# patello/azul_deep_reinforcement_learning

Hardware: AMD Instinct MI355X
Metric: Azul env steps/sec (random-agent self-play), bit-exact vs CPU (higher is better)
Workload: dtype u8/u32 (+f64 sampling)

## Files before the change

### azul_deep_reinforcement_learning_amd/csrc/azul_common.hpp

```cpp
#pragma once
#include <stdint.h>

typedef uint32_t u32;
typedef int32_t  i32;
typedef uint64_t u64;
typedef int64_t  i64;

#if !defined(__HIPCC__)
#error "libazulhip's headers are gfx950 device code: compile with hipcc --offload-arch=gfx950"
#endif
#include <hip/hip_runtime.h>
#define AZ_FN __device__ __forceinline__
#define AZ_MEMBER_FN __attribute__((device)) __forceinline__
#define AZ_UNLIKELY(x) __builtin_expect(!!(x), 0)

namespace wv {
AZ_FN u32 lane() { return __builtin_amdgcn_mbcnt_hi(~0u, __builtin_amdgcn_mbcnt_lo(~0u, 0u)); }

template <class A, class B> struct same_type { static constexpr bool value = false; };
template <class A> struct same_type<A, A> { static constexpr bool value = true; };
constexpr bool LOCKSTEP_EMULATION = same_type<decltype(__builtin_amdgcn_s_memtime()), unsigned long long>::value;
template <int SIMM16> struct HwReg { static constexpr int value = SIMM16; };
template <class R> AZ_FN u32 getreg(R)
{
    if constexpr (LOCKSTEP_EMULATION) return 0u;
    else return __builtin_amdgcn_s_getreg(R::value);
}
AZ_FN u32 hw_id() { return getreg(HwReg<(4 | (31 << 11))>()); }
AZ_FN u32 hw_xcc_id() { return getreg(HwReg<(20 | (31 << 11))>()); }
constexpr int PRIO_BLOCK = 128;
AZ_FN void set_prio(bool hi) { if (hi) __builtin_amdgcn_s_setprio(1); else __builtin_amdgcn_s_setprio(0); }
}

namespace az {

enum { ST_OK = 0, ST_ILLEGAL_MOVE = 1, ST_GAME_ENDED = 2, ST_STUCK = 3, ST_BAD_ACTION = 4, ST_BOX_EMPTY = 5,
       ST_TRUNCATED = 6  };
enum { POOL_RANDOM = 0, POOL_LID = 1 };
#ifndef AZ_DRAW_MARGIN
#define AZ_DRAW_MARGIN 8192ull
#endif
enum { T_ROWS = 31, T_BINADES = 8, T_STRIDE = 9 , T_PAIRS = T_ROWS * T_STRIDE };

enum { SEG_MASK = 0, SEG_SAMPLE, SEG_MOVE, SEG_AFTERMOVE, SEG_TAIL, SEG_NEWROUND, SEG_SCORE, SEG_RESET, SEG_LOOP, SEG_COUNT };
constexpr int AZ_PROF_SLOTS = 48;
enum { WCNT_ROUND_END = 0, WCNT_DEAL, WCNT_RESET, WCNT_COUNT };
constexpr int AZ_WAVE_REC_WORDS = 8;
#if defined(AZ_PROFILE_SEGMENTS)
struct SegProf { u64 last; u64 acc[SEG_COUNT]; u32 cnt[WCNT_COUNT]; };
#define AZ_COUNT(which, cond) do { if (prof_) prof_->cnt[which] += (u32)__popcll(__builtin_amdgcn_ballot_w64(cond)) >> 5; } while (0)
struct WaveStamps { u64 entry, loop_start, loop_end; };
#define AZ_WAVE_STAMP(field) (wstamps.field = __builtin_amdgcn_s_memtime())
#define AZ_STAMP(seg) do { if (prof_) { u64 now_ = __builtin_amdgcn_s_memtime(); prof_->acc[seg] += now_ - prof_->last; prof_->last = now_; } } while (0)
#else
struct SegProf { int unused; };
#define AZ_STAMP(seg) do { } while (0)
#define AZ_COUNT(which, cond) do { } while (0)
#define AZ_WAVE_STAMP(field) do { } while (0)
#endif

struct Rules {
    u32 first_player;
    u32 tile_pool;
};

constexpr u32 column_board_c(int col)
{
    u32 m = 0;
    for (int j = 0; j < 5; j++) m |= 1u << (5 * j + ((col - j + 5) % 5));
    return m;
}
static_assert(column_board_c(0) == 0x222201u && column_board_c(4) == 0x111110u, "column boards");

AZ_FN i32 floor_penalty(u32 floor_tiles)
{
// ... 53 lines not shown
```

### azul_deep_reinforcement_learning_amd/csrc/azul_kernels.hip

```cpp
#include <hip/hip_runtime.h>
#include <math.h>
#include <stdio.h>
#include <stdlib.h>
#include <string.h>

#include <mutex>
#include <string>
#include <vector>

#include "../../include/azul_hip.h"
#include "azul_common.hpp"
#include "azul_tables.hpp"

using namespace az;

#include "azul_selfplay_kernels.hpp"

#include "azul_x_kernels.hpp"

#include "azul_policy.hpp"
#include "azul_rollout2.hpp"
#include "azul_learner.hpp"

struct azul_batch {
// ... 78 lines not shown
    for (void *p : bufs) if (p) (void)hipFree(p);
    if (b->ev0) (void)hipEventDestroy(b->ev0);
    if (b->ev1) (void)hipEventDestroy(b->ev1);
    for (hipEvent_t e : b->lev) (void)hipEventDestroy(e);
    if (b->call_pin) (void)hipHostFree(b->call_pin);
    delete b;
}

static int batch_alloc(azul_batch *b, int n_games, int first_player, int tile_pool)
{
    HIP_TRY(hipGetDevice(&b->device));
    const size_t N = (size_t)n_games;
    const size_t RB = (size_t)b->rec_bytes;
    b->d.n = (u32)n_games;
    b->d.rules.first_player = (u32)first_player;
    b->d.rules.tile_pool = (u32)tile_pool;
    b->d.draw_margin = AZ_DRAW_MARGIN;
    HIP_TRY(hipMalloc((void **)&b->d.state, N * RB));
    HIP_TRY(hipMalloc((void **)&b->d.mt, N * 624 * sizeof(u32)));
    HIP_TRY(hipMalloc((void **)&b->d.mtpos, N * sizeof(u32)));
    HIP_TRY(hipMalloc((void **)&b->d.episodes, N * sizeof(u64)));
    HIP_TRY(hipMalloc((void **)&b->d.stuck, N * sizeof(u32)));
    HIP_TRY(hipMalloc((void **)&b->d.stat_sum, N * 10 * sizeof(double)));
    HIP_TRY(hipMalloc((void **)&b->d.prof, AZ_PROF_SLOTS * sizeof(u64)));
    HIP_TRY(hipMemset(b->d.prof, 0, AZ_PROF_SLOTS * sizeof(u64)));
#if defined(AZ_PROFILE_SEGMENTS)
    HIP_TRY(hipMalloc((void **)&b->d.wave_prof, (N + 1) / 2 * AZ_WAVE_REC_WORDS * sizeof(u64)));
    HIP_TRY(hipMemset(b->d.wave_prof, 0, (N + 1) / 2 * AZ_WAVE_REC_WORDS * sizeof(u64)));
#endif
    {
        const int rows = 5 * (b->displays + 1) + 1;
        std::vector<double> hX((size_t)rows * T_STRIDE * 2);
        if (!build_sample_pairs(rows, hX.data())) return fail(AZUL_ERR_INVALID, "weight-table decomposition check failed on this host");
        HIP_TRY(hipMalloc((void **)&b->Tx, hX.size() * sizeof(double)));
        HIP_TRY(hipMemcpy(b->Tx, hX.data(), hX.size() * sizeof(double), hipMemcpyHostToDevice));
        b->d.tab = (const double2 *)b->Tx;
    }
    HIP_TRY(hipMemset(b->d.state, 0, N * RB));
    HIP_TRY(hipMemset(b->d.mt, 0, N * 624 * sizeof(u32)));
    {
        std::vector<u32> pos(N, 624u);
        HIP_TRY(hipMemcpy(b->d.mtpos, pos.data(), N * sizeof(u32), hipMemcpyHostToDevice));
    }
    HIP_TRY(hipMemset(b->d.episodes, 0, N * sizeof(u64)));
    HIP_TRY(hipMemset(b->d.stuck, 0, N * sizeof(u32)));
    HIP_TRY(hipMemset(b->d.stat_sum, 0, N * 10 * sizeof(double)));
    HIP_TRY(hipEventCreate(&b->ev0));
    HIP_TRY(hipEventCreate(&b->ev1));
    return AZUL_SUCCESS;
}

int azul_batch_create(azul_batch_t **out, int n_games, int first_player, int tile_pool)
{
    return azul_batch_create_players(out, n_games, 2, first_player, tile_pool);
}

int azul_batch_create_players(azul_batch_t **out, int n_games, int players, int first_player, int tile_pool)
{
    return azul_batch_create_rules(out, n_games, players, first_player, tile_pool, 0u);
}

int azul_batch_create_rules(azul_batch_t **out, int n_games, int players, int first_player, int tile_pool, unsigned rule_flags)
{
    if (!out || n_games <= 0) return fail(AZUL_ERR_INVALID, "azul_batch_create: bad arguments");
    if (players < 2 || players > 4) return fail(AZUL_ERR_INVALID, "players must be 2, 3 or 4");
    if (first_player < 0 || first_player > players) return fail(AZUL_ERR_RULE, "first_player must be 0 (Random) or 1 .. players");
// ... 1410 lines not shown
```

### azul_deep_reinforcement_learning_amd/csrc/azul_rules_x.hpp

```cpp
#pragma once
#include "azul_selfplay2.hpp"
#include "azul_env2.hpp"

namespace azx {
using namespace az;
using namespace az2;

enum { XPOOL_RANDOM = 0, XPOOL_LID = 1, XPOOL_BAG = 2 };

struct RulesX {
    u32 first_player;
    u32 pool;
    u32 end_bonus;
    u32 short_deal;
};

template <u32 D>
struct Dim {
    static constexpr u32 S = D + 1;
    static constexpr u32 Q = 5 * S;
    static constexpr u32 NA = 6 * Q;
    static constexpr u32 NW = Q > 32 ? 2 : 1;
    static constexpr u32 NL = (NA + 63) / 64;
    static constexpr u32 TROWS = Q + 1;
// ... 611 lines not shown
            if (o.action) o.action[o.e] = av;
            if (o.reward) o.reward[o.e] = 0;
            if (o.packed) o.packed[o.e] = pk;
            if (o.done) o.done[o.e] = (uint8_t)dn;
        }
        if (o.rec) gx_store(g, o.rec + o.e * (u32)AZUL_RECORD_BYTES_WIDE, l);
    }
}

template <u32 P, u32 D, int OUT, bool PAD, bool BITS>
AZ_FN u32 selfplay_step_x(GX<P, D> &g, const RulesX &rules, const KX<D> &K, Rng2 &r, const Tab2 &T, u64 margin, Counters2 &cnt,
                          const Out2 &o, bool &dead, SegProf *prof_ = nullptr)
{
    (void)prof_;
    AZ_STAMP(SEG_LOOP);
    const K2 &k = K.k;
    const u32 l = k.l;
    const bool hard = r.pos + 2u > 624u;
    u32 wa, wb;
    {
        const u32 i = hard ? 622u : r.pos;
        wa = r.tlds[i]; wb = r.tlds[i + 1u];
    }
    MaskX<D> m;
    legal_mask_x(g, K, m);
    u32 pre[7];
    pre[0] = 0;
#pragma unroll
    for (u32 rr = 0; rr < 6u; rr++) pre[rr + 1] = pre[rr] + row_count<D>(m, rr);
    const u32 J = pre[1], L = pre[6];
    const bool nomove = (L == 0u) | (g.eog != 0u);
    const u32 M = L - J, Mc = M ? M : 256u, Jc = J < Dim<D>::TROWS ? J : Dim<D>::TROWS - 1u;
    const u32 kbase = M ? J : 0u;
    const double u01 = ((double)(wa >> 5) * 67108864.0 + (double)(wb >> 6)) * (1.0 / 9007199254740992.0);
    const double2 fs = T.fs[9u * Jc + 31u - (u32)__builtin_clz(Mc)];
    if (OUT == 1 || (OUT == 2 && o.mask)) store_mask_x<D, (PAD && OUT == 1)>(o, m, l);
    if ((OUT == 1 && BITS) || (OUT == 2 && o.maskbits)) store_maskbits_x<D>(o, m, l);
    AZ_STAMP(SEG_MASK);
    const double sJ = fs.y;
    const double total = ((double)M + fs.x) + 0.0;
    double u = u01;
    double x = u * total;
    double d = x - sJ;
    u32 fl = (u32)d;
    double fr = d - (double)fl;
    u32 kg = kbase + fl + 1u;
    bool edge = !(__builtin_fabs(fr - 0.5) < 0.5 - 1e-9) | (kg > L);
    r.pos += 2u;
    bool any_nomove = false;
    if (AZ_UNLIKELY(wave_any(hard | edge | nomove))) {
        r.pos -= (hard | nomove) ? 2u : 0u;
        if (hard & !nomove) {
            const bool one = r.pos == 623u;
            const u32 last = r.tlds[623];
            lds_sync();
            rng2_twist(r, l);
            const u32 t0 = r.tlds[0], t1 = r.tlds[1];
            wa = one ? last : t0; wb = one ? t0 : t1;
            r.pos = one ? 1u : 2u;
            u = ((double)(wa >> 5) * 67108864.0 + (double)(wb >> 6)) * (1.0 / 9007199254740992.0);
            x = u * total;
            d = x - sJ; fl = (u32)d; fr = d - (double)fl;
            kg = kbase + fl + 1u;
            edge = !(__builtin_fabs(fr - 0.5) < 0.5 - 1e-9) | (kg > L);
        }
        if (edge & !nomove) {
            const double sT = M ? sJ : T.fs[9u * Jc].y;
            kg = sample_slow2(T, M ? x : u * (sT + 0.0), sT, J, M, L);
        }
        any_nomove = wave_any(nomove);
    }
    Choice<D> ch;
    pick_action_x<D>(m, pre, kg, k, ch);
    AZ_STAMP(SEG_SAMPLE);

    u32 ret = 0;
    if (AZ_UNLIKELY(any_nomove)) {
        if (nomove) {
            cnt.stuck_add += 1u;
            {
                MaskX<D> none;
#pragma unroll
                for (u32 rr = 0; rr < 6u; rr++)
#pragma unroll
                    for (u32 ww = 0; ww < Dim<D>::NW; ww++) { none.m[rr][ww] = 0u; none.bit[rr][ww] = 0u; }
                if (OUT == 1 || (OUT == 2 && o.mask)) store_mask_x<D, (PAD && OUT == 1)>(o, none, l);
                if ((OUT == 1 && BITS) || (OUT == 2 && o.maskbits)) store_maskbits_x<D>(o, none, l);
            }
            outputs_x<P, D, OUT>(g, o, -1, 2u, l);
            const u32 st0 = restart_x(g, rules, r, margin, K);
            ret = st0 ? (0x100u | st0) : 2u;
        }
        dead |= (ret & 0x100u) != 0u;
        AZ_STAMP(SEG_RESET);
    }
    if (!nomove) {
        do_move_x(g, ch.s, ch.c, ch.row, rules.pool != (u32)XPOOL_RANDOM, K);
        sources_x(g);
        AZ_STAMP(SEG_MOVE);
        const bool eor = (g.B0 | g.B1) == 0u;
        g.cur = eor ? g.cur : (g.cur < P ? g.cur + 1u : 1u);
        u32 st = ST_OK;
// ... 77 lines not shown
struct XOp {
    int op;
    const i32 *actions;
    const uint8_t *active;
    const uint8_t *mask_in;
    i32 *actions_out;
    uint8_t *status;
    uint8_t *mask;
    float *obs;
    int persp;
    uint8_t *flags;
    double *stats;
    uint8_t *player;
    uint8_t *rng_dirty;
    uint8_t *rec_out;
    u32 *pos_out;
    i32 *next_action;
    u32 pos_set;
    u32 first, count;
};

struct XTraj {
    int n_steps;
    uint8_t *mask; u64 *maskbits; i32 *action; i32 *reward; uint8_t *done; uint8_t *rec; u32 *packed;
    u32 mask_stride;
};

AZ_FN bool xop_draws(int op) { return op == XOP_INIT || op == XOP_NEW_ROUND || op == XOP_STEP || op == XOP_RANDOM_ACTION || op == XOP_SAMPLE_MASK; }

template <u32 D>
AZ_FN void stage_tab_x(const double2 *tab, double2 *tab_lds, u32 lane)
{
    for (u32 i = lane; i < Dim<D>::TROWS * (u32)T_STRIDE; i += 64u) tab_lds[i] = tab[i];
    lds_sync();
}

template <u32 D>
AZ_FN void store_mask_bytes_x(const MaskX<D> &m, uint8_t *row, u32 l)
{
    row += l;
#pragma unroll
    for (u32 rr = 0; rr < 6u; rr++) {
        if (l < (Dim<D>::Q < 32u ? Dim<D>::Q : 32u)) row[Dim<D>::Q * rr] = (uint8_t)m.bit[rr][0];
        if (Dim<D>::NW > 1) { if (l < Dim<D>::Q - 32u) row[Dim<D>::Q * rr + 32u] = (uint8_t)m.bit[rr][Dim<D>::NW - 1]; }
    }
}

template <u32 P, u32 D>
AZ_FN void open_game_x(GX<P, D> &g, KX<D> &K, const uint8_t *rec, u32 l)
{
    kx_init(K);
    gx_load(g, rec, l);
    prime_x(g, K);
}

AZ_FN void open_stream_x(Rng2 &r, Counters2 &cnt, const XBatchDev &b, u32 gi, u32 *lds, u32 l)
{
    rng2_open(r, b.mt + (size_t)gi * 624u, lds, b.mtpos[gi], l);
    counters2_open(cnt, b.episodes + gi, b.stuck + gi, b.stat_sum + (size_t)gi * 10, l);
}
AZ_FN void close_stream_x(Rng2 &r, const Counters2 &cnt, const XBatchDev &b, u32 gi, u32 l)
{
    rng2_close(r, b.mt + (size_t)gi * 624u, b.mtpos + gi, l);
    counters2_close(cnt, l);
}

// ... 77 lines not shown
        if (dirty_state) gx_store(g, rec, l);
        if (a.next_action && use_rng && st == ST_OK && r.pos + 2u <= 624u) {
            const u32 keep = r.pos;
            MaskX<D> m;
            legal_mask_x(g, K, m);
            spec = random_agent_x<D>(m, r, tab, K.k);
            r.pos = keep;
        }
        if (use_rng) rng2_close(r, gmt, b.mtpos + gi, l);
        rdirty = r.dirty;
    }
    if (a.next_action && l == 0u) a.next_action[oi] = spec;
    if (a.rng_dirty && l == 0u) a.rng_dirty[oi] = (uint8_t)rdirty;
    if (a.status && act && l == 0u) a.status[oi] = (uint8_t)st;
    if (a.rec_out) gx_store(g, a.rec_out + (size_t)oi * AZUL_RECORD_BYTES_WIDE, l);
    if (a.pos_out && l == 0u) a.pos_out[oi] = b.mtpos[gi];
    if (a.mask) {
        MaskX<D> m;
        legal_mask_x(g, K, m);
        store_mask_bytes_x<D>(m, a.mask + (size_t)oi * Dim<D>::NA, l);
    }
    if (a.obs) observe_x(g, (u32)a.persp < P ? (u32)a.persp : mex(g), a.obs + (size_t)oi * obs_size<P, D>(), l);
    if (a.flags) {
        const u32 f = ((g.B0 | g.B1) == 0u ? AZUL_FLAG_END_OF_ROUND : 0) | (g.over ? AZUL_FLAG_END_OF_GAME : 0) | (g.eog ? AZUL_FLAG_ENDED_FLAG : 0);
        if (l == 0u) a.flags[oi] = (uint8_t)f;
    }
    if (a.stats) {
        if (l == 0u) for (u32 q = 0; q < 10u; q++) a.stats[(size_t)oi * 10 + q] = game_stat_x(g, q);
    }
    if (a.player && l == 0u) a.player[oi] = (uint8_t)g.cur;
}

template <u32 P, u32 D, int OUT, bool PAD, bool BITS>
AZ_FN void selfplay_body_x(const XBatchDev &b, const XTraj &t, u32 wave_id, u32 (*mt_lds)[624], u32 (*mtt_lds)[624], double2 *tab_lds)
{
    const u32 lane = wv::lane(), l = lane & 31u, half = lane >> 5;
    stage_tab_x<D>(b.tab, tab_lds, lane);
    const u32 gi = wave_id * 2u + half;
    if (gi >= b.n) return;
    uint8_t *rec = b.state + (size_t)gi * AZUL_RECORD_BYTES_WIDE;
    KX<D> K;
    const Tab2 tab = {tab_lds};
    GX<P, D> g;
    open_game_x(g, K, rec, l);
    Rng2 r;
    u32 *gmt = b.mt + (size_t)gi * 624u;
    rng2_open(r, gmt, mt_lds[half], b.mtpos[gi], l);
    rng2_attach_tempered(r, mtt_lds[half], l);
    Counters2 cnt;
    counters2_open(cnt, b.episodes + gi, b.stuck + gi, b.stat_sum + (size_t)gi * 10, l);
    Out2 o = {t.mask, t.maskbits, t.action, t.reward, t.done, t.packed, t.rec, t.mask_stride, gi,
              l == 0u ? (u32 *)t.action : (l == 1u ? (u32 *)t.reward : t.packed)};
    bool dead = false;
#if defined(AZ_PROFILE_SEGMENTS)
    SegProf prof;
    for (int q = 0; q < SEG_COUNT; q++) prof.acc[q] = 0;
    prof.last = __builtin_amdgcn_s_memtime();
    SegProf *pp = &prof;
#else
    SegProf *pp = nullptr;
#endif
    u32 turn = wv::hw_id() & 1u;
#pragma unroll 1
    for (int s0 = 0; s0 < t.n_steps; s0 += wv::PRIO_BLOCK) {
        wv::set_prio(turn != 0u);
        turn ^= 1u;
        const int s1 = s0 + wv::PRIO_BLOCK < t.n_steps ? s0 + wv::PRIO_BLOCK : t.n_steps;
#pragma unroll 1
        for (int s = s0; s < s1; s++) {
            if (!dead) selfplay_step_x<P, D, OUT, PAD, BITS>(g, b.rules, K, r, tab, b.draw_margin, cnt, o, dead, pp);
            else {
                cnt.stuck_add += 1u;
                {
                    MaskX<D> none;
#pragma unroll
// ... 447 lines not shown
```

### azul_deep_reinforcement_learning_amd/csrc/azul_selfplay2.hpp

```cpp
#pragma once
#include "azul_common.hpp"

namespace az2 {
using namespace az;

AZ_FN u32 wlane() { return wv::lane(); }
AZ_FN bool upper() { return (wlane() & 32u) != 0u; }
AZ_FN u32 hsel(u64 b) { return upper() ? (u32)(b >> 32) : (u32)b; }
AZ_FN u32 hb(bool p) { return hsel(__builtin_amdgcn_ballot_w64(p)); }
AZ_FN u32 hread(u32 v, u32 idx) { return (u32)__builtin_amdgcn_ds_bpermute((int)((idx << 2) | ((wlane() & 32u) << 2)), (int)v); }
AZ_FN u32 hbcast(u32 v, u32 idx) { return hread(v, idx); }
AZ_FN u32 hread4(u32 v, u32 idx, u32 h4) { return (u32)__builtin_amdgcn_ds_bpermute((int)((idx << 2) | h4), (int)v); }
template <u32 IDX>
AZ_FN u32 hbcast_c(u32 v)
{
    u32 a = (u32)__builtin_amdgcn_readlane((int)v, (int)IDX), b = (u32)__builtin_amdgcn_readlane((int)v, (int)(IDX + 32u));
    return upper() ? b : a;
}
AZ_FN bool wave_any(bool p) { return __builtin_amdgcn_ballot_w64(p) != 0ull; }
AZ_FN double hread_d(double v, u32 idx)
{
    u64 b = (u64)__double_as_longlong(v);
    u32 lo = hread((u32)b, idx), hi = hread((u32)(b >> 32), idx);
    return __longlong_as_double((long long)(((u64)hi << 32) | lo));
// ... 271 lines not shown
}
#endif

struct Mask2 {
    u32 m[6];
    u32 bit[6];
    u32 B;
};

AZ_FN u32 ok_board2(u32 cp, u32 wall, const K2 &k)
{
    const u32 l = k.l;
    const u32 pme = hb(cp != 0u) & 0x1ffffffu;
    const u32 rb = (pme >> (k.prow * 5u)) & 31u;
    const u32 bad = (rb & ~(1u << k.pcol)) | ((wall >> l) & 1u);
    return hb(bad == 0u) & 0x1ffffffu;
}

AZ_FN void legal_mask2(const G2 &g, const K2 &k, Mask2 &out)
{
    const u32 B = g.B;
    const u32 has = (B >> k.spos) & 1u;
    const u32 okc = (me2(g) ? g.ok1 : g.ok0) >> k.col6;
    out.B = B;
    out.bit[0] = has;
    out.m[0] = hb(has != 0u);
#pragma unroll
    for (u32 w = 1; w < 6u; w++) {
        out.bit[w] = has & (okc >> (5u * (w - 1u)));
        out.m[w] = hb((out.bit[w] & 1u) != 0u);
    }
}

struct Tab2 { const double2 *fs; };

AZ_FN double tpat2(const Tab2 &t, u32 J, u32 m) { return (double)m + t.fs[9u * J + 31u - (u32)__builtin_clz(m)].x; }
AZ_FN double tseq2(const Tab2 &t, u32 J, u32 kk) { return kk <= J ? t.fs[9u * kk].y : tpat2(t, J, kk - J); }

AZ_FN u32 sample_slow2(const Tab2 &T, double x, double sJ, u32 J, u32 M, u32 L)
{
    const bool floors = x < sJ;
    const double y = floors ? x * 100.0 : x - sJ;
    const u32 fy = (u32)y;
    const u32 cap = floors ? J : M;
    const u32 g = fy + 1u > cap ? cap : fy + 1u;
    u32 kg = floors ? g : J + g;
    const bool exact = floors & (__builtin_fabs((y - (double)fy) - 0.5) < 0.5 - 1e-9);
    for (u32 it = exact ? 256u : 0u; it < 256u; it++) {
        if (kg > 1u && x < tseq2(T, J, kg - 1u)) kg -= 1u;
        else if (kg < L && !(x < tseq2(T, J, kg))) kg += 1u;
        else break;
    }
    return kg;
}

template <bool LID>
AZ_FN bool do_move2f(G2 &g, u32 src, u32 db, u32 c, u32 row, bool from_display, u32 B , const K2 &k)
{
    const u32 l = k.l;
    const u32 me = me2(g);
    const u32 cell = 5u * ((row ? row : 1u) - 1u) + c;
    u32 mine = me ? g.cp1 : g.cp0;
    const u32 n = hread4(g.cs, src, k.h4);
    const u32 moved = hread4(g.cs, l - 25u + db, k.h4);
    const u32 old = hread4(mine, cell, k.h4);
    bool token = (!from_display) & (((B >> 30) & 1u) != 0u);
    bool centre = (l >= 25u) & (l < 30u) & (l != 25u + c) & from_display;
    bool gone = ((l >= db) & (l < db + 5u) & from_display) | (l == src) | ((l == 30u) & token);
    const u32 grown = g.cs + (centre ? moved : 0u);
    g.cs = gone ? 0u : grown;
    g.nfp = token ? g.cur : g.nfp;
    u32 fl = (me ? g.floor1 : g.floor0) + (token ? 1u : 0u);
    i32 overflow = row ? (i32)row - (i32)old - (i32)n : -(i32)n;
    u32 spill = overflow < 0 ? (u32)(-overflow) : 0u;
    u32 newv = overflow < 0 ? row : old + n;
    mine = ((l == cell) & (row != 0u)) ? newv : mine;
    g.cp0 = me ? g.cp0 : mine;
    g.cp1 = me ? mine : g.cp1;
    {
        const u32 sh = 5u * ((row ? row : 1u) - 1u);
        u32 okm = me ? g.ok1 : g.ok0;
        okm = row ? ((okm & ~(31u << sh)) | (1u << (sh + c))) : okm;
        g.ok0 = me ? g.ok0 : okm;
        g.ok1 = me ? okm : g.ok1;
// ... 471 lines not shown
            u32 st2 = episode_reset2<LID>(g, first_player, r, margin, k);
            if (st2) ret = 0x100u | st2;
        }
        dead |= (ret & 0x100u) != 0u;
        AZ_STAMP(SEG_RESET);
    }
    return ret;
}

template <bool LID, int OUT, bool PAD, bool BITS, bool LIM = false>
AZ_FN u32 selfplay_step2(G2 &g, u32 first_player, const K2 &k, Rng2 &r, const Tab2 &T, u64 margin, Counters2 &cnt, const Out2 &o,
                        SegProf *prof_, bool &dead )
{
    (void)prof_;
    AZ_STAMP(SEG_LOOP);
    const u32 l = k.l;
    const bool hard = r.pos + 2u > 624u;
    u32 wa, wb;
    {
        const u32 i = hard ? 622u : r.pos;
        wa = r.tlds[i]; wb = r.tlds[i + 1u];
    }

    Mask2 m;
    legal_mask2(g, k, m);
    const u32 c0 = __popc(m.m[0]), c1 = __popc(m.m[1]), c2 = __popc(m.m[2]), c3 = __popc(m.m[3]), c4 = __popc(m.m[4]), c5 = __popc(m.m[5]);
    const u32 J = c0;
    const u32 p1 = c0, p2 = p1 + c1, p3 = p2 + c2, p4 = p3 + c3, p5 = p4 + c4, L = p5 + c5;
    const bool nomove = (L == 0u) | (g.eog != 0u);
    const u32 M = L - J;
    const u32 Jc = J < 31u ? J : 30u;
    const u32 Mc = M ? M : 256u;
    const u32 kbase = M ? J : 0u;
    const double u01 = ((double)(wa >> 5) * 67108864.0 + (double)(wb >> 6)) * (1.0 / 9007199254740992.0);
    __builtin_amdgcn_sched_barrier(0);
    const double2 fs = T.fs[9u * Jc + 31u - (u32)__builtin_clz(Mc)];
    __builtin_amdgcn_sched_barrier(0);
    if (OUT == 1 || (OUT == 2 && o.mask))
        store_mask_row2<(PAD && OUT == 1)>(o, m.m[0], m.m[1], m.m[2], m.m[3], m.m[4], m.m[5], m.bit[0], m.bit[1], m.bit[2], m.bit[3], m.bit[4], m.bit[5], l);
    if ((OUT == 1 && BITS) || (OUT == 2 && o.maskbits)) {
        const u64 q0 = (u64)m.m[0] | ((u64)m.m[1] << 30) | ((u64)m.m[2] << 60);
        const u64 q1 = ((u64)m.m[2] >> 4) | ((u64)m.m[3] << 26) | ((u64)m.m[4] << 56);
        const u64 q2 = ((u64)m.m[4] >> 8) | ((u64)m.m[5] << 22);
        const u32 q = l < 2u ? l : 2u;
        o.maskbits[o.e * 3u + q] = q == 0u ? q0 : (q == 1u ? q1 : q2);
    }
    __builtin_amdgcn_sched_barrier(0);
    AZ_STAMP(SEG_MASK);
    const double sJ = fs.y;
    const double total = ((double)M + fs.x) + 0.0;
    double u = u01;
    double x = u * total;
    double d = x - sJ;
    u32 fl = (u32)d;
    double fr = d - (double)fl;
    u32 kg = kbase + fl + 1u;
    bool edge = !(__builtin_fabs(fr - 0.5) < 0.5 - 1e-9) | (kg > L);
    r.pos += 2u;
    bool any_nomove = false;
    if (AZ_UNLIKELY(wave_any(hard | edge | nomove))) {
        r.pos -= (hard | nomove) ? 2u : 0u;
        if (hard & !nomove) {
            const bool one = r.pos == 623u;
            const u32 last = r.tlds[623];
            lds_sync();
            rng2_twist(r, l);
            const u32 t0 = r.tlds[0], t1 = r.tlds[1];
            wa = one ? last : t0; wb = one ? t0 : t1;
            r.pos = one ? 1u : 2u;
            u = ((double)(wa >> 5) * 67108864.0 + (double)(wb >> 6)) * (1.0 / 9007199254740992.0);
            x = u * total;
            d = x - sJ; fl = (u32)d; fr = d - (double)fl;
            kg = kbase + fl + 1u;
            edge = !(__builtin_fabs(fr - 0.5) < 0.5 - 1e-9) | (kg > L);
        }
        if (edge & !nomove) {
            const double sT = M ? sJ : T.fs[9u * Jc].y;
            kg = sample_slow2(T, M ? x : u * (sT + 0.0), sT, J, M, L);
        }
        any_nomove = wave_any(nomove);
    }
    const u32 want = kg - 1u;
    const bool g1 = want >= p1, g2 = want >= p2, g3 = want >= p3, g4 = want >= p4, g5 = want >= p5;
    const u32 w01 = g1 ? m.m[1] : m.m[0], w23 = g3 ? m.m[3] : m.m[2], w45 = g5 ? m.m[5] : m.m[4];
    const u32 b01 = g1 ? p1 : 0u, b23 = g3 ? p3 : p2, b45 = g5 ? p5 : p4;
    const u32 mword = g4 ? w45 : (g2 ? w23 : w01);
    const u32 base = g4 ? b45 : (g2 ? b23 : b01);
    const u32 prow_ = (u32)g1 + (u32)g2 + (u32)g3 + (u32)g4 + (u32)g5;
    const bool hit = (((u32)__popc(mword & ((1u << l) - 1u)) - (want - base)) << 1) + ((mword >> l) & 1u) == 1u;
    const u32 who = hb(hit);
    const u32 ln = (u32)__builtin_ctz(who | 0x80000000u);
    const u32 ac = (ln * 43u) >> 8, ad = ln - 6u * ac;
    const bool a_disp = ad != 0u;
    const u32 a_db = a_disp ? 5u * ad - 5u : 0u;
    const u32 a_src = a_disp ? a_db + ac : 25u + ac;
    const i32 a = (i32)(30u * prow_ + ln);
    AZ_STAMP(SEG_SAMPLE);

    u32 ret = 0;
    if (AZ_UNLIKELY(any_nomove)) {
        if (nomove) {
            cnt.stuck_add += 1u;
            outputs2<OUT>(g, o, -1, 0, 2u, l);
            u32 st0 = episode_reset2<LID>(g, first_player, r, margin, k);
            ret = st0 ? (0x100u | st0) : 2u;
        }
        dead |= (ret & 0x100u) != 0u;
        AZ_STAMP(SEG_RESET);
    }
    if (!nomove) {
        const u32 me = me2(g);
        const bool filled = do_move2f<LID>(g, a_src, a_db, ac, prow_, a_disp, m.B, k);
// ... 22 lines not shown
```

### azul_deep_reinforcement_learning_amd/csrc/azul_selfplay_kernels.hpp

```cpp
#pragma once
#include "azul_ops2.hpp"

__global__ void __launch_bounds__(64) azul_seed_kernel(BatchDev b, u64 seed_base, const u64 *seeds)
{
    u32 g = blockIdx.x * 64u + threadIdx.x;
    if (g >= b.n) return;
    u64 seed = seeds ? seeds[g] : seed_base + (u64)g;
    seed_stream(b.mt + (size_t)g * 624u, seed);
    b.mtpos[g] = 624u;
}

template <bool LID>
__global__ void __launch_bounds__(64) azul_op_kernel(BatchDev b, OpArgs a)
{
    __shared__ u32 mt_lds[2][az2::MT_LDS_WORDS];
    __shared__ double2 tabfs_lds[T_PAIRS];
    __shared__ float obs_lds[2][OP2_OBS_STRIDE];
    op_body2<LID>(b, a, blockIdx.x, mt_lds, tabfs_lds, obs_lds);
}

template <bool LID>
__global__ void __launch_bounds__(64) azul_score_moves_kernel(BatchDev b, ScoreMovesArgs a)
{
    az2::score_moves_body2<LID>(b, a, blockIdx.x);
// ... 134 lines not shown
            w |= ((m & 0xffu) != 0u ? 1u : 0u) << (4u * j);
            w |= ((m & 0xff00u) != 0u ? 1u : 0u) << (4u * j + 1u);
            w |= ((m & 0xff0000u) != 0u ? 1u : 0u) << (4u * j + 2u);
            w |= ((m & 0xff000000u) != 0u ? 1u : 0u) << (4u * j + 3u);
        }
    } else if (d == 40u) {
        const i32 av = a.action[cell];
        w = (av < 0 ? 0xffu : (u32)av & 0xffu) | ((u32)a.done[cell] << 8) | ((u32)a.player[cell] << 16);
    } else if (d == 41u) w = (u32)a.reward[cell];
    else {
        const float *src = d == 42u ? a.value : d == 43u ? a.logp : d == 44u ? a.entropy : a.returns;
        w = __builtin_bit_cast(u32, src[cell]);
    }
    a.out[i] = w;
}

struct TrajArgs {
    int n_steps;
    uint8_t *mask;
    u64 *maskbits;
    i32 *action;
    i32 *reward;
    uint8_t *done;
    uint8_t *rec;
    u32 *packed;
};


template <bool LID, int OUT, bool PAD, bool BITS, bool LIM = false >
__global__ void __launch_bounds__(64) azul_selfplay2_kernel(BatchDev b, TrajArgs t, u32 mask_stride)
{
    __shared__ u32 mt_lds[2][az2::MT_LDS_WORDS];
    __shared__ u32 mtt_lds[2][624];
    __shared__ double2 tabfs_lds[T_PAIRS];
#if defined(AZ_PROFILE_SEGMENTS)
    WaveStamps wstamps;
#endif
    AZ_WAVE_STAMP(entry);
    const u32 lane = wv::lane(), l = lane & 31u, half = lane >> 5;
    for (u32 i = lane; i < (u32)T_PAIRS; i += 64u) tabfs_lds[i] = b.tab[i];
    az2::lds_sync();
    const u32 nb = gridDim.x, xcd = blockIdx.x & 7u, q8 = nb >> 3, rem = nb & 7u;
    const u32 wave_id = xcd * q8 + (xcd < rem ? xcd : rem) + (blockIdx.x >> 3);
    const u32 gi = wave_id * 2u + half;
    if (gi >= b.n) return;
    uint8_t *rec = b.state + (size_t)gi * AZUL_RECORD_BYTES;
    az2::K2 k;
    az2::k2_init(k);
    az2::rng2_set_move_limit(mt_lds[half], b.move_limit, l);
    az2::Tab2 tab = {tabfs_lds};
    az2::G2 g;
    az2::g2_load(g, rec, l);
    az2::prime2(g, k);
    az2::Rng2 r;
    u32 *gmt = b.mt + (size_t)gi * 624u;
    az2::rng2_open(r, gmt, mt_lds[half], b.mtpos[gi], l);
    az2::rng2_attach_tempered(r, mtt_lds[half], l);
    const u64 margin = b.draw_margin;
    az2::Counters2 cnt;
    az2::counters2_open(cnt, b.episodes + gi, b.stuck + gi, b.stat_sum + (size_t)gi * 10, l);
    az2::Out2 o = {t.mask, t.maskbits, t.action, t.reward, t.done, t.packed, t.rec, mask_stride, gi,
                   l == 0u ? (u32 *)t.action : (l == 1u ? (u32 *)t.reward : t.packed)};
#if defined(AZ_PROFILE_SEGMENTS)
    SegProf prof;
    for (int q = 0; q < SEG_COUNT; q++) prof.acc[q] = 0;
    for (int q = 0; q < WCNT_COUNT; q++) prof.cnt[q] = 0;
    prof.last = AZ_WAVE_STAMP(loop_start);
    SegProf *pp = &prof;
#else
    SegProf *pp = nullptr;
#endif
    bool dead = false;
    u32 turn = wv::hw_id() & 1u;
    if (LIM) {
        u32 skipped = 0;
#pragma unroll 1
        for (int s0 = 0; s0 < t.n_steps; s0 += wv::PRIO_BLOCK) {
            wv::set_prio(turn != 0u);
            turn ^= 1u;
            const int s1 = s0 + wv::PRIO_BLOCK < t.n_steps ? s0 + wv::PRIO_BLOCK : t.n_steps;
#pragma unroll 1
            for (int s = s0; s < s1; s++) {
                if (!dead) az2::selfplay_step2<LID, OUT, PAD, BITS, true>(g, b.rules.first_player, k, r, tab, margin, cnt, o, pp, dead);
// ... 49 lines not shown
```

### azul_deep_reinforcement_learning_amd/csrc/azul_tables.hpp

```cpp
#pragma once
#include "azul_common.hpp"

namespace az {

static inline void build_weight_table(double *T )
{
    double s = 0.0;
    for (int J = 0; J < 31; J++) {
        if (J > 0) s = s + 0.01;
        double c = s;
        T[J * 151] = c;
        for (int m = 1; m < 151; m++) { c = c + 1.0; T[J * 151 + m] = c; }
    }
}

static inline bool build_sample_pairs(int rows, double *out )
{
    const int mmax = 5 * (rows - 1);
    bool ok = mmax < 256;
    double s = 0.0;
    for (int J = 0; J < rows; J++) {
        if (J > 0) s = s + 0.01;
        double fr[8] = {0, 0, 0, 0, 0, 0, 0, 0};
        double c = s;
        for (int m = 1; m <= mmax; m++) {
            c = c + 1.0;
            const int b = 31 - __builtin_clz((unsigned)m);
            if (m == (1 << b)) fr[b] = c - (double)m;
            if ((double)m + fr[b] != c) ok = false;
        }
        for (int b = 0; b < 8; b++) { out[2 * (9 * J + b)] = fr[b]; out[2 * (9 * J + b) + 1] = s; }
        out[2 * (9 * J + 8)] = 100.0 * s;
        out[2 * (9 * J + 8) + 1] = 0.0;
    }
    return ok;
}

}
```

### azul_deep_reinforcement_learning_amd/csrc/azul_x_kernels.hpp

```cpp
#pragma once
#include "azul_rules_x.hpp"

template <u32 P, u32 D>
__global__ void __launch_bounds__(64) azul_x_op_kernel(azx::XBatchDev b, azx::XOp a)
{
    __shared__ u32 mt_lds[2][624];
    __shared__ double2 tab_lds[azx::Dim<D>::TROWS * T_STRIDE];
    azx::op_body_x<P, D>(b, a, blockIdx.x, mt_lds, tab_lds);
}

template <u32 P, u32 D, int OUT, bool PAD, bool BITS>
__global__ void __launch_bounds__(64) azul_x_selfplay_kernel(azx::XBatchDev b, azx::XTraj t)
{
    __shared__ u32 mt_lds[2][624];
    __shared__ u32 mtt_lds[2][624];
    __shared__ double2 tab_lds[azx::Dim<D>::TROWS * T_STRIDE];
    const u32 nb = gridDim.x, xcd = blockIdx.x & 7u, q8 = nb >> 3, rem = nb & 7u;
    const u32 wave_id = xcd * q8 + (xcd < rem ? xcd : rem) + (blockIdx.x >> 3);
    azx::selfplay_body_x<P, D, OUT, PAD, BITS>(b, t, wave_id, mt_lds, mtt_lds, tab_lds);
}

template <u32 P, u32 D>
__global__ void __launch_bounds__(64) azul_x_runner_kernel(azx::XBatchDev b, azx::XRun a)
{
    __shared__ u32 mt_lds[2][624];
    __shared__ double2 tab_lds[azx::Dim<D>::TROWS * T_STRIDE];
    azx::runner_body_x<P, D>(b, a, blockIdx.x, mt_lds, tab_lds);
}

template <u32 P, u32 D>
__global__ void __launch_bounds__(64) azul_x_net_kernel(azx::XBatchDev b, azx::XNet a)
{
    __shared__ u32 mt_lds[2][624];
    azx::net_body_x<P, D>(b, a, blockIdx.x, mt_lds);
}

template <u32 P, u32 D>
__global__ void __launch_bounds__(64) azul_x_score_moves_kernel(azx::XBatchDev b, azx::XScoreMoves a)
{
    azx::score_moves_body_x<P, D>(b, a, blockIdx.x);
}

template <u32 P_, u32 D_>
struct XShape { static constexpr u32 P = P_, D = D_; };

template <class F>
static auto x_for_shape(int players, int displays, F f) -> decltype(f(XShape<2, 5>()))
{
    const int pd = players * 16 + displays;
    if (pd == 2 * 16 + 5) return f(XShape<2, 5>());
    if (pd == 3 * 16 + 5) return f(XShape<3, 5>());
    if (pd == 3 * 16 + 7) return f(XShape<3, 7>());
    if (pd == 4 * 16 + 5) return f(XShape<4, 5>());
    if (pd == 4 * 16 + 9) return f(XShape<4, 9>());
    return nullptr;
}

typedef void (*x_selfplay_kernel_t)(azx::XBatchDev, azx::XTraj);
template <u32 P, u32 D>
static x_selfplay_kernel_t x_selfplay_kernel_of(SelfplayVariant v)
{
    if (v.out == 0) return azul_x_selfplay_kernel<P, D, 0, false, false>;
    if (v.out == 1 && v.pad && v.bits) return azul_x_selfplay_kernel<P, D, 1, true, true>;
    if (v.out == 1 && v.pad) return azul_x_selfplay_kernel<P, D, 1, true, false>;
    return azul_x_selfplay_kernel<P, D, 2, false, false>;
}
static x_selfplay_kernel_t x_selfplay_kernel(int players, int displays, SelfplayVariant v)
{
    return x_for_shape(players, displays, [&](auto s) { return x_selfplay_kernel_of<s.P, s.D>(v); });
}
```

Measured before the change: 3.149 billion.

## Replace f64 move sampling with 32-bit fixed-point fast path plus exact fallback

Move sampling in the selfplay kernels now uses a 24-bit fractional fixed-point table in LDS, built from the f64 table at kernel start. It takes the index from a single umulhi instead of several f64 multiplies and conversions. Draws that land within a small margin of a bucket boundary are flagged as edge cases and sent to an exact f64 path that reads the global table, so results stay bit-exact. The fixed-point table also halves LDS use for the table. The cost is a somewhat higher edge-case rate, and the slow path now makes global-memory reads.

```diff
diff --git a/azul_deep_reinforcement_learning_amd/csrc/azul_common.hpp b/azul_deep_reinforcement_learning_amd/csrc/azul_common.hpp
--- a/azul_deep_reinforcement_learning_amd/csrc/azul_common.hpp
+++ b/azul_deep_reinforcement_learning_amd/csrc/azul_common.hpp
@@ -41,6 +41,14 @@
 #define AZ_DRAW_MARGIN 8192ull
 #endif
 enum { T_ROWS = 31, T_BINADES = 8, T_STRIDE = 9 , T_PAIRS = T_ROWS * T_STRIDE };
+
+struct alignas(8) PairQ { u32 t, s; };
+enum { TQ_FRAC = 24, TQ_MARGIN = 8 };
+__host__ __device__ __forceinline__ PairQ sample_pair_q(double t, double s)
+{
+    PairQ q = {(u32)(t * 16777216.0), (u32)(s * 16777216.0 + 0.5)};
+    return q;
+}
 
 enum { SEG_MASK = 0, SEG_SAMPLE, SEG_MOVE, SEG_AFTERMOVE, SEG_TAIL, SEG_NEWROUND, SEG_SCORE, SEG_RESET, SEG_LOOP, SEG_COUNT };
 constexpr int AZ_PROF_SLOTS = 48;
diff --git a/azul_deep_reinforcement_learning_amd/csrc/azul_kernels.hip b/azul_deep_reinforcement_learning_amd/csrc/azul_kernels.hip
--- a/azul_deep_reinforcement_learning_amd/csrc/azul_kernels.hip
+++ b/azul_deep_reinforcement_learning_amd/csrc/azul_kernels.hip
@@ -134,6 +134,7 @@
         const int rows = 5 * (b->displays + 1) + 1;
         std::vector<double> hX((size_t)rows * T_STRIDE * 2);
         if (!build_sample_pairs(rows, hX.data())) return fail(AZUL_ERR_INVALID, "weight-table decomposition check failed on this host");
+        if (!sample_pairs_q_from(rows, hX.data(), nullptr)) return fail(AZUL_ERR_INVALID, "fixed-point weight-table range check failed on this host");
         HIP_TRY(hipMalloc((void **)&b->Tx, hX.size() * sizeof(double)));
         HIP_TRY(hipMemcpy(b->Tx, hX.data(), hX.size() * sizeof(double), hipMemcpyHostToDevice));
         b->d.tab = (const double2 *)b->Tx;
diff --git a/azul_deep_reinforcement_learning_amd/csrc/azul_rules_x.hpp b/azul_deep_reinforcement_learning_amd/csrc/azul_rules_x.hpp
--- a/azul_deep_reinforcement_learning_amd/csrc/azul_rules_x.hpp
+++ b/azul_deep_reinforcement_learning_amd/csrc/azul_rules_x.hpp
@@ -667,20 +667,14 @@
     const bool nomove = (L == 0u) | (g.eog != 0u);
     const u32 M = L - J, Mc = M ? M : 256u, Jc = J < Dim<D>::TROWS ? J : Dim<D>::TROWS - 1u;
     const u32 kbase = M ? J : 0u;
-    const double u01 = ((double)(wa >> 5) * 67108864.0 + (double)(wb >> 6)) * (1.0 / 9007199254740992.0);
-    const double2 fs = T.fs[9u * Jc + 31u - (u32)__builtin_clz(Mc)];
+    const u32 U = draw_top32(wa, wb);
+    const u32 ti = 9u * Jc + 31u - (u32)__builtin_clz(Mc);
+    const PairQ tq = T.q[ti];
     if (OUT == 1 || (OUT == 2 && o.mask)) store_mask_x<D, (PAD && OUT == 1)>(o, m, l);
     if ((OUT == 1 && BITS) || (OUT == 2 && o.maskbits)) store_maskbits_x<D>(o, m, l);
     AZ_STAMP(SEG_MASK);
-    const double sJ = fs.y;
-    const double total = ((double)M + fs.x) + 0.0;
-    double u = u01;
-    double x = u * total;
-    double d = x - sJ;
-    u32 fl = (u32)d;
-    double fr = d - (double)fl;
-    u32 kg = kbase + fl + 1u;
-    bool edge = !(__builtin_fabs(fr - 0.5) < 0.5 - 1e-9) | (kg > L);
+    bool edge;
+    u32 kg = sample_fixed2(U, tq, M, kbase, L, edge);
     r.pos += 2u;
     bool any_nomove = false;
     if (AZ_UNLIKELY(wave_any(hard | edge | nomove))) {
@@ -693,16 +687,9 @@
             const u32 t0 = r.tlds[0], t1 = r.tlds[1];
             wa = one ? last : t0; wb = one ? t0 : t1;
             r.pos = one ? 1u : 2u;
-            u = ((double)(wa >> 5) * 67108864.0 + (double)(wb >> 6)) * (1.0 / 9007199254740992.0);
-            x = u * total;
-            d = x - sJ; fl = (u32)d; fr = d - (double)fl;
-            kg = kbase + fl + 1u;
-            edge = !(__builtin_fabs(fr - 0.5) < 0.5 - 1e-9) | (kg > L);
-        }
-        if (edge & !nomove) {
-            const double sT = M ? sJ : T.fs[9u * Jc].y;
-            kg = sample_slow2(T, M ? x : u * (sT + 0.0), sT, J, M, L);
-        }
+            kg = sample_fixed2(draw_top32(wa, wb), tq, M, kbase, L, edge);
+        }
+        if (edge & !nomove) kg = sample_exact2(T, wa, wb, ti, J, Jc, M, kbase, L);
         any_nomove = wave_any(nomove);
     }
     Choice<D> ch;
@@ -846,6 +833,15 @@
 AZ_FN void stage_tab_x(const double2 *tab, double2 *tab_lds, u32 lane)
 {
     for (u32 i = lane; i < Dim<D>::TROWS * (u32)T_STRIDE; i += 64u) tab_lds[i] = tab[i];
+    lds_sync();
+}
+template <u32 D>
+AZ_FN void stage_tabq_x(const double2 *tab, PairQ *tabq_lds, u32 lane)
+{
+    for (u32 i = lane; i < Dim<D>::TROWS * (u32)T_STRIDE; i += 64u) {
+        const double2 p = tab[i];
+        tabq_lds[i] = sample_pair_q(p.x, p.y);
+    }
     lds_sync();
 }
 
@@ -989,15 +985,15 @@
 }
 
 template <u32 P, u32 D, int OUT, bool PAD, bool BITS>
-AZ_FN void selfplay_body_x(const XBatchDev &b, const XTraj &t, u32 wave_id, u32 (*mt_lds)[624], u32 (*mtt_lds)[624], double2 *tab_lds)
+AZ_FN void selfplay_body_x(const XBatchDev &b, const XTraj &t, u32 wave_id, u32 (*mt_lds)[624], u32 (*mtt_lds)[624], PairQ *tabq_lds)
 {
     const u32 lane = wv::lane(), l = lane & 31u, half = lane >> 5;
-    stage_tab_x<D>(b.tab, tab_lds, lane);
+    stage_tabq_x<D>(b.tab, tabq_lds, lane);
     const u32 gi = wave_id * 2u + half;
     if (gi >= b.n) return;
     uint8_t *rec = b.state + (size_t)gi * AZUL_RECORD_BYTES_WIDE;
     KX<D> K;
-    const Tab2 tab = {tab_lds};
+    const Tab2 tab = {b.tab, tabq_lds};
     GX<P, D> g;
     open_game_x(g, K, rec, l);
     Rng2 r;
diff --git a/azul_deep_reinforcement_learning_amd/csrc/azul_selfplay2.hpp b/azul_deep_reinforcement_learning_amd/csrc/azul_selfplay2.hpp
--- a/azul_deep_reinforcement_learning_amd/csrc/azul_selfplay2.hpp
+++ b/azul_deep_reinforcement_learning_amd/csrc/azul_selfplay2.hpp
@@ -327,7 +327,20 @@
     }
 }
 
-struct Tab2 { const double2 *fs; };
+struct Tab2 {
+    const double2 *fs;
+    const PairQ *q = nullptr;
+};
+
+AZ_FN u32 draw_top32(u32 wa, u32 wb) { return (wa & 0xffffffe0u) | (wb >> 27); }
+AZ_FN u32 sample_fixed2(u32 U, PairQ q, u32 M, u32 kbase, u32 L, bool &edge)
+{
+    const u32 Tq = (M << TQ_FRAC) + q.t;
+    const u32 D = __umulhi(U, Tq) - q.s;
+    const u32 kg = kbase + (D >> TQ_FRAC) + 1u;
+    edge = (((D + (u32)TQ_MARGIN) & 0xffffffu) < 2u * (u32)TQ_MARGIN) | (kg > L);
+    return kg;
+}
 
 AZ_FN double tpat2(const Tab2 &t, u32 J, u32 m) { return (double)m + t.fs[9u * J + 31u - (u32)__builtin_clz(m)].x; }
 AZ_FN double tseq2(const Tab2 &t, u32 J, u32 kk) { return kk <= J ? t.fs[9u * kk].y : tpat2(t, J, kk - J); }
@@ -345,6 +358,24 @@
         if (kg > 1u && x < tseq2(T, J, kg - 1u)) kg -= 1u;
         else if (kg < L && !(x < tseq2(T, J, kg))) kg += 1u;
         else break;
+    }
+    return kg;
+}
+
+AZ_FN u32 sample_exact2(const Tab2 &T, u32 wa, u32 wb, u32 ti, u32 J, u32 Jc, u32 M, u32 kbase, u32 L)
+{
+    const double2 fs = T.fs[ti];
+    const double sJ = fs.y;
+    const double total = ((double)M + fs.x) + 0.0;
+    const double u = ((double)(wa >> 5) * 67108864.0 + (double)(wb >> 6)) * (1.0 / 9007199254740992.0);
+    const double x = u * total;
+    const double d = x - sJ;
+    const u32 fl = (u32)d;
+    const double fr = d - (double)fl;
+    u32 kg = kbase + fl + 1u;
+    if (!(__builtin_fabs(fr - 0.5) < 0.5 - 1e-9) | (kg > L)) {
+        const double sT = M ? sJ : T.fs[9u * Jc].y;
+        kg = sample_slow2(T, M ? x : u * (sT + 0.0), sT, J, M, L);
     }
     return kg;
 }
@@ -882,9 +913,10 @@
     const u32 Jc = J < 31u ? J : 30u;
     const u32 Mc = M ? M : 256u;
     const u32 kbase = M ? J : 0u;
-    const double u01 = ((double)(wa >> 5) * 67108864.0 + (double)(wb >> 6)) * (1.0 / 9007199254740992.0);
+    const u32 U = draw_top32(wa, wb);
+    const u32 ti = 9u * Jc + 31u - (u32)__builtin_clz(Mc);
     __builtin_amdgcn_sched_barrier(0);
-    const double2 fs = T.fs[9u * Jc + 31u - (u32)__builtin_clz(Mc)];
+    const PairQ tq = T.q[ti];
     __builtin_amdgcn_sched_barrier(0);
     if (OUT == 1 || (OUT == 2 && o.mask))
         store_mask_row2<(PAD && OUT == 1)>(o, m.m[0], m.m[1], m.m[2], m.m[3], m.m[4], m.m[5], m.bit[0], m.bit[1], m.bit[2], m.bit[3], m.bit[4], m.bit[5], l);
@@ -897,15 +929,8 @@
     }
     __builtin_amdgcn_sched_barrier(0);
     AZ_STAMP(SEG_MASK);
-    const double sJ = fs.y;
-    const double total = ((double)M + fs.x) + 0.0;
-    double u = u01;
-    double x = u * total;
-    double d = x - sJ;
-    u32 fl = (u32)d;
-    double fr = d - (double)fl;
-    u32 kg = kbase + fl + 1u;
-    bool edge = !(__builtin_fabs(fr - 0.5) < 0.5 - 1e-9) | (kg > L);
+    bool edge;
+    u32 kg = sample_fixed2(U, tq, M, kbase, L, edge);
     r.pos += 2u;
     bool any_nomove = false;
     if (AZ_UNLIKELY(wave_any(hard | edge | nomove))) {
@@ -918,16 +943,9 @@
             const u32 t0 = r.tlds[0], t1 = r.tlds[1];
             wa = one ? last : t0; wb = one ? t0 : t1;
             r.pos = one ? 1u : 2u;
-            u = ((double)(wa >> 5) * 67108864.0 + (double)(wb >> 6)) * (1.0 / 9007199254740992.0);
-            x = u * total;
-            d = x - sJ; fl = (u32)d; fr = d - (double)fl;
-            kg = kbase + fl + 1u;
-            edge = !(__builtin_fabs(fr - 0.5) < 0.5 - 1e-9) | (kg > L);
+            kg = sample_fixed2(draw_top32(wa, wb), tq, M, kbase, L, edge);
         }
-        if (edge & !nomove) {
-            const double sT = M ? sJ : T.fs[9u * Jc].y;
-            kg = sample_slow2(T, M ? x : u * (sT + 0.0), sT, J, M, L);
-        }
+        if (edge & !nomove) kg = sample_exact2(T, wa, wb, ti, J, Jc, M, kbase, L);
         any_nomove = wave_any(nomove);
     }
     const u32 want = kg - 1u;
diff --git a/azul_deep_reinforcement_learning_amd/csrc/azul_selfplay_kernels.hpp b/azul_deep_reinforcement_learning_amd/csrc/azul_selfplay_kernels.hpp
--- a/azul_deep_reinforcement_learning_amd/csrc/azul_selfplay_kernels.hpp
+++ b/azul_deep_reinforcement_learning_amd/csrc/azul_selfplay_kernels.hpp
@@ -190,13 +190,16 @@
 {
     __shared__ u32 mt_lds[2][az2::MT_LDS_WORDS];
     __shared__ u32 mtt_lds[2][624];
-    __shared__ double2 tabfs_lds[T_PAIRS];
+    __shared__ PairQ tabq_lds[T_PAIRS];
 #if defined(AZ_PROFILE_SEGMENTS)
     WaveStamps wstamps;
 #endif
     AZ_WAVE_STAMP(entry);
     const u32 lane = wv::lane(), l = lane & 31u, half = lane >> 5;
-    for (u32 i = lane; i < (u32)T_PAIRS; i += 64u) tabfs_lds[i] = b.tab[i];
+    for (u32 i = lane; i < (u32)T_PAIRS; i += 64u) {
+        const double2 p = b.tab[i];
+        tabq_lds[i] = sample_pair_q(p.x, p.y);
+    }
     az2::lds_sync();
     const u32 nb = gridDim.x, xcd = blockIdx.x & 7u, q8 = nb >> 3, rem = nb & 7u;
     const u32 wave_id = xcd * q8 + (xcd < rem ? xcd : rem) + (blockIdx.x >> 3);
@@ -206,7 +209,7 @@
     az2::K2 k;
     az2::k2_init(k);
     az2::rng2_set_move_limit(mt_lds[half], b.move_limit, l);
-    az2::Tab2 tab = {tabfs_lds};
+    az2::Tab2 tab = {b.tab, tabq_lds};
     az2::G2 g;
     az2::g2_load(g, rec, l);
     az2::prime2(g, k);
diff --git a/azul_deep_reinforcement_learning_amd/csrc/azul_tables.hpp b/azul_deep_reinforcement_learning_amd/csrc/azul_tables.hpp
--- a/azul_deep_reinforcement_learning_amd/csrc/azul_tables.hpp
+++ b/azul_deep_reinforcement_learning_amd/csrc/azul_tables.hpp
@@ -36,4 +36,25 @@
     return ok;
 }
 
+static inline bool sample_pairs_q_from(int rows, const double *pairs , u32 *out )
+{
+    bool ok = rows >= 1 && 5 * (rows - 1) < 256;
+    for (int i = 0; i < rows * 9 && ok; i++) {
+        const double t = pairs[2 * i], s = pairs[2 * i + 1];
+        const bool floor_only = i % 9 == 8;
+        ok = t >= 0.0 && t < (floor_only ? 256.0 : 1.0) && s >= 0.0 && s < 1.0 && (!floor_only || s == 0.0);
+        if (ok && out) { const PairQ q = sample_pair_q(t, s); out[2 * i] = q.t; out[2 * i + 1] = q.s; }
+    }
+    return ok;
 }
+
+static inline bool build_sample_pairs_q(int rows, u32 *out )
+{
+    if (rows < 1 || 5 * (rows - 1) >= 256) return false;
+    double *d = new double[(size_t)rows * 9 * 2];
+    const bool ok = build_sample_pairs(rows, d) && sample_pairs_q_from(rows, d, out);
+    delete[] d;
+    return ok;
+}
+
+}
diff --git a/azul_deep_reinforcement_learning_amd/csrc/azul_x_kernels.hpp b/azul_deep_reinforcement_learning_amd/csrc/azul_x_kernels.hpp
--- a/azul_deep_reinforcement_learning_amd/csrc/azul_x_kernels.hpp
+++ b/azul_deep_reinforcement_learning_amd/csrc/azul_x_kernels.hpp
@@ -14,10 +14,10 @@
 {
     __shared__ u32 mt_lds[2][624];
     __shared__ u32 mtt_lds[2][624];
-    __shared__ double2 tab_lds[azx::Dim<D>::TROWS * T_STRIDE];
+    __shared__ PairQ tabq_lds[azx::Dim<D>::TROWS * T_STRIDE];
     const u32 nb = gridDim.x, xcd = blockIdx.x & 7u, q8 = nb >> 3, rem = nb & 7u;
     const u32 wave_id = xcd * q8 + (xcd < rem ? xcd : rem) + (blockIdx.x >> 3);
-    azx::selfplay_body_x<P, D, OUT, PAD, BITS>(b, t, wave_id, mt_lds, mtt_lds, tab_lds);
+    azx::selfplay_body_x<P, D, OUT, PAD, BITS>(b, t, wave_id, mt_lds, mtt_lds, tabq_lds);
 }
 
 template <u32 P, u32 D>
@@ -65,7 +65,8 @@
     if (v.out == 1 && v.pad) return azul_x_selfplay_kernel<P, D, 1, true, false>;
     return azul_x_selfplay_kernel<P, D, 2, false, false>;
 }
-static x_selfplay_kernel_t x_selfplay_kernel(int players, int displays, SelfplayVariant v)
+template <class V>
+static x_selfplay_kernel_t x_selfplay_kernel(int players, int displays, V v)
 {
     return x_for_shape(players, displays, [&](auto s) { return x_selfplay_kernel_of<s.P, s.D>(v); });
 }
```

Result: no change. 3.180 billion (median of 6 runs) (+1.0%).
